# amolrpatil21/PorQua

Measured on AMD Instinct MI355X. Metric: QPs solved/sec (rebalance dates) at N=1000 assets, 1-8 GPU; x vs host CPU, higher is better.
Workload: dtype f64; 1 GPU; config3: long-only min-variance (P=2*Pearson cov, budget + box [0,1]), daily rebalance; n_assets=1000, window=252, dates_per_gpu=4749, global_batch=4749, parallelism=dates-sharded x1

## Files before the change

porqua_amd/csrc/common.h:

```cpp
#pragma once
#include <hip/hip_runtime.h>
#include <stdint.h>

#ifndef PQ_DEVFN
#define PQ_DEVFN __device__ __forceinline__
#endif

namespace pq {

typedef double f64x4 __attribute__((ext_vector_type(4)));

constexpr int TB = 64;
constexpr int KC = 16;
constexpr int LDW = 80;
constexpr int STAGE = KC * LDW;
constexpr int NTHR = 256;

struct Acc {
  f64x4 c[2][2];
  __device__ __forceinline__ void zero() {
#pragma unroll
    for (int m = 0; m < 2; ++m)
#pragma unroll
      for (int n = 0; n < 2; ++n) c[m][n] = f64x4{0.0, 0.0, 0.0, 0.0};
// ... 60 lines not shown
  for (int e = 0; e < 4; ++e) S[(k + e) * LDW + i] = s.v[e];
}

enum { MODE_KI = 0, MODE_IK = 1 };

template <int MA, int MB>
__device__ __forceinline__ void stage_load(Stage4& sa, Stage4& sb, const double* GA, int64_t lda,
                                           int a_i0, const double* GB, int64_t ldb, int b_j0,
                                           int k0, int ka0, int kb0) {
  if (MA == MODE_KI) load_ki(sa, GA, lda, ka0 + k0, a_i0); else load_ik(sa, GA, lda, ka0 + k0, a_i0);
  if (MB == MODE_KI) load_ki(sb, GB, ldb, kb0 + k0, b_j0); else load_ik(sb, GB, ldb, kb0 + k0, b_j0);
}
template <int MA, int MB>
__device__ __forceinline__ void stage_store(const Stage4& sa, const Stage4& sb, double* SA, double* SB) {
  if (MA == MODE_KI) store_ki(sa, SA); else store_ik(sa, SA);
  if (MB == MODE_KI) store_ki(sb, SB); else store_ik(sb, SB);
}

template <int MA, int MB>
__device__ void gemm_stream(Acc& acc, double* lds, const double* GA, int64_t lda, int a_i0, int ka0,
                            const double* GB, int64_t ldb, int b_j0, int kb0, int K) {
  if (K <= 0) return;
  Stage4 ra, rb;
  __syncthreads();
  stage_load<MA, MB>(ra, rb, GA, lda, a_i0, GB, ldb, b_j0, 0, ka0, kb0);
  stage_store<MA, MB>(ra, rb, lds, lds + STAGE);
  __syncthreads();
  int buf = 0;
  for (int k0 = 0; k0 < K; k0 += KC) {
    const bool more = (k0 + KC) < K;
    if (more) stage_load<MA, MB>(ra, rb, GA, lda, a_i0, GB, ldb, b_j0, k0 + KC, ka0, kb0);
    mma_lds(acc, lds + buf * 2 * STAGE, lds + buf * 2 * STAGE + STAGE, KC);
    if (more) stage_store<MA, MB>(ra, rb, lds + (buf ^ 1) * 2 * STAGE, lds + (buf ^ 1) * 2 * STAGE + STAGE);
    __syncthreads();
    buf ^= 1;
  }
}

__device__ __forceinline__ void acc_to_lds(const Acc& acc, double* T, int ldt, double alpha) {
#pragma unroll
  for (int m = 0; m < 2; ++m)
#pragma unroll
    for (int n = 0; n < 2; ++n)
#pragma unroll
      for (int r = 0; r < 4; ++r) T[acc_row(m, r) * ldt + acc_col(n)] = alpha * acc.c[m][n][r];
}
__device__ __forceinline__ void acc_to_lds_T(const Acc& acc, double* S, double alpha) {
#pragma unroll
  for (int m = 0; m < 2; ++m)
#pragma unroll
    for (int n = 0; n < 2; ++n)
#pragma unroll
      for (int r = 0; r < 4; ++r) S[acc_col(n) * LDW + acc_row(m, r)] = alpha * acc.c[m][n][r];
}

__device__ __forceinline__ void acc_store(const Acc& acc, double* G, int64_t ld, int row0, int col0) {
#pragma unroll
  for (int m = 0; m < 2; ++m)
#pragma unroll
    for (int n = 0; n < 2; ++n)
#pragma unroll
      for (int r = 0; r < 4; ++r)
        G[(int64_t)(row0 + acc_row(m, r)) * ld + col0 + acc_col(n)] = acc.c[m][n][r];
}
__device__ __forceinline__ void acc_store_T(const Acc& acc, double* G, int64_t ld, int row0, int col0) {
#pragma unroll
  for (int m = 0; m < 2; ++m)
#pragma unroll
    for (int n = 0; n < 2; ++n)
#pragma unroll
      for (int r = 0; r < 4; ++r)
        G[(int64_t)(row0 + acc_col(n)) * ld + col0 + acc_row(m, r)] = acc.c[m][n][r];
}

__device__ __forceinline__ int loop_zero() {
  int z;
  asm volatile("s_mov_b32 %0, 0" : "=s"(z));
  return z;
}

__device__ __forceinline__ double readlane_f64(double v, int lane) {
  const int lo = __builtin_amdgcn_readlane(__double2loint(v), lane);
  const int hi = __builtin_amdgcn_readlane(__double2hiint(v), lane);
  return __hiloint2double(hi, lo);
}

template <int K>
__device__ __forceinline__ double row_bcast16_k(double v) {
  const int lo = __builtin_amdgcn_update_dpp(0, __double2loint(v), 0x150 + K, 0xF, 0xF, false);
  const int hi = __builtin_amdgcn_update_dpp(0, __double2hiint(v), 0x150 + K, 0xF, 0xF, false);
  return __hiloint2double(hi, lo);
}
__device__ __forceinline__ double row_bcast16(double v, int k) {
  switch (k) {
    case 0: return row_bcast16_k<0>(v);
    case 1: return row_bcast16_k<1>(v);
    case 2: return row_bcast16_k<2>(v);
    case 3: return row_bcast16_k<3>(v);
    case 4: return row_bcast16_k<4>(v);
    case 5: return row_bcast16_k<5>(v);
    case 6: return row_bcast16_k<6>(v);
    case 7: return row_bcast16_k<7>(v);
    case 8: return row_bcast16_k<8>(v);
    case 9: return row_bcast16_k<9>(v);
    case 10: return row_bcast16_k<10>(v);
    case 11: return row_bcast16_k<11>(v);
    case 12: return row_bcast16_k<12>(v);
    case 13: return row_bcast16_k<13>(v);
    case 14: return row_bcast16_k<14>(v);
    default: return row_bcast16_k<15>(v);
  }
}


__device__ __forceinline__ int wave_chol_inv16(double (&A)[4], double (&Bv)[4], const int l) {
  const int cc = l & 15, gg = l >> 4;
  int bad = 0;
#pragma unroll
  for (int kk = 0; kk < 16; ++kk) {
    const int src = ((kk & 3) << 4);
    const double akk = A[kk >> 2];
    const double piv = readlane_f64(akk, src | kk);
    const double rowk = __shfl(akk, src | cc, 64);
    const double bkr = __shfl(Bv[kk >> 2], src | cc, 64);
    double colv[4];
#pragma unroll
    for (int q = 0; q < 4; ++q) colv[q] = row_bcast16(A[q], kk);
    if (!(piv > 0.0) || !isfinite(piv)) bad = 1;
    double rs = __builtin_amdgcn_rsq(piv);
    rs = rs * fma(-0.5 * piv * rs, rs, 1.5);
    rs = rs * fma(-0.5 * piv * rs, rs, 1.5);
    const double bk = bkr * rs;
    const double lck = cc > kk ? rowk * rs : 0.0;
#pragma unroll
    for (int q = 0; q < 4; ++q) {
      if (4 * q + 3 < kk) continue;
      const int r = gg + 4 * q;
      const double lrk = colv[q] * rs;
      const double lrt = r > kk ? lrk : 0.0;
      const double upd = fma(-lrt, lck, A[q]);
      A[q] = (cc == kk && r >= kk) ? lrk : upd;
      const double bu = fma(-lrt, bk, Bv[q]);
      Bv[q] = r == kk ? bk : bu;
    }
  }
  return bad;
}
__device__ __forceinline__ int wave_chol_inv16(double (&A)[4], double (&Bv)[4]) {
  return wave_chol_inv16(A, Bv, lane_id());
}

__device__ __forceinline__ int xcd_slot(int g, int N) {
  const int x = g & 7, q = N >> 3, r = N & 7;
  return (x < r ? x * (q + 1) : r * (q + 1) + (x - r) * q) + (g >> 3);
}

template <int W>
__device__ __forceinline__ double lanes_sum(double v) {
  static_assert(W >= 2 && W <= 64 && (W & (W - 1)) == 0, "a power of two, at most the wave");
#pragma unroll
  for (int o = W / 2; o > 0; o >>= 1) v += __shfl_xor(v, o, 64);
  return v;
}
template <int W>
__device__ __forceinline__ double lanes_max(double v) {
  static_assert(W >= 2 && W <= 64 && (W & (W - 1)) == 0, "a power of two, at most the wave");
#pragma unroll
  for (int o = W / 2; o > 0; o >>= 1) v = fmax(v, __shfl_xor(v, o, 64));
  return v;
}
__device__ __forceinline__ double wave_sum(double v) { return lanes_sum<64>(v); }
__device__ __forceinline__ double wave_max(double v) { return lanes_max<64>(v); }

__device__ __forceinline__ double block_sum(double v, double* red) {
  v = wave_sum(v);
  const int nw = blockDim.x >> 6;
  __syncthreads();
  if (lane_id() == 0) red[wave_id()] = v;
  __syncthreads();
  double s = 0.0;
  for (int w = 0; w < nw; ++w) s += red[w];
  return s;
}
__device__ __forceinline__ double block_max(double v, double* red) {
  v = wave_max(v);
  const int nw = blockDim.x >> 6;
  __syncthreads();
  if (lane_id() == 0) red[wave_id()] = v;
  __syncthreads();
  double s = red[0];
  for (int w = 1; w < nw; ++w) s = fmax(s, red[w]);
  return s;
}

}
```

porqua_amd/csrc/pg_record.h:

```cpp
#pragma once
#include "common.h"
#include "../../include/porqua_hip.h"

namespace pq {

constexpr int PGR = PQ_PG_RECORD;
enum : int {
  R_K = 0, R_MA = 1, R_NZB = 2, R_STATE = 3, R_ROUNDS = 4, R_SC = 5,
  R_FORMED = 6, R_REUSE = 7,
  R_ACT = 64, R_LAM = 128, R_DA = 192, R_SOL = 256, R_AL = 288,
  R_W = 320, R_NFX = 321, R_FIX = 324, R_FIXV = 332, R_FXL = 340,
  R_GFORM = 348,
  R_KB = 349,
  R_LIST = 352, R_CNT = 360
};
constexpr int PG_NBUCKET = 6;
constexpr int PG_BIGB = 5;
__device__ __forceinline__ unsigned long long pg_count(const double* rec, int bk) {
  return reinterpret_cast<const unsigned long long*>(rec + R_CNT)[bk];
}
__device__ __forceinline__ int pg_listed(const double* rec, int bk, int i) {
  return (int)rec[(int64_t)i * PGR + R_LIST + bk];
}
int resident_grid(const void* kernel, int block, int B);
__device__ __forceinline__ int pg_bucket(int kb) {
  return kb <= 48 ? 0 : kb <= 64 ? 1 : kb <= 80 ? 2 : kb <= 96 ? 3 : 4;
}
constexpr int PG_KMAX = 128;
constexpr int PG_KBIG = 256;
constexpr int PG_MGMAX = 32;
constexpr int PG_WMB = 8;
constexpr int PG_WG_MAX = 24;
static_assert(R_FXL + PG_WMB <= R_GFORM && R_KB < R_LIST && R_LIST + 6 <= R_CNT && R_CNT + 6 <= PQ_PG_RECORD,
              "PQ_PG_RECORD too small");

struct PGWork {
  double *xs, *xb, *g, *Px, *rF, *solx, *pxb, *U;
  int *Fl, *fl, *posF;
  __device__ __forceinline__ PGWork(const pq_state& st, int b, int ld) {
    double* W = st.work + (int64_t)b * st.work_stride;
    xs = W;
    xb = W + ld;
    g = W + 2 * (int64_t)ld;
    Px = W + 3 * (int64_t)ld;
    Fl = reinterpret_cast<int*>(W + 4 * (int64_t)ld);
    posF = Fl + ld;
    rF = W + 5 * (int64_t)ld;
    solx = W + 6 * (int64_t)ld;
    pxb = W + 7 * (int64_t)ld;
    U = W + 8 * (int64_t)ld;
    fl = reinterpret_cast<int*>(U + (int64_t)st.mg_pad * ld);
  }
};

__device__ __forceinline__ int pk(int r, int c) { return ((r * (r + 1)) >> 1) + c; }

}

int pq_pg_solve_rt_launch(int nbmax, int B, hipStream_t str, const pq_problem* pb, pq_state* st, double* rec,
                          const pq_settings* s, int ldk);
int pq_pg_wide_launch(const pq_lowrank* lr, const pq_problem* pb, pq_state* st, double* rec, const pq_settings* s,
                      const pq_pg_wide* wd, hipStream_t stream);
```

porqua_amd/csrc/polish_g.hip:

```cpp
#include <cstdlib>
#include <mutex>

#include "polish_dev.h"
#include "capi_util.h"
#include "pg_record.h"

namespace pq {


__global__ __launch_bounds__(PT) void k_pg_init(pq_lowrank lr, pq_problem pb, pq_state st, double* rec,
                                                pq_settings s) {
  __shared__ double red[16];
  const int b = blockIdx.x;
  const int t = threadIdx.x;
  double* R = rec + (int64_t)b * PGR;
  const int st0 = st.status[b];
  if (st0 != PQ_SOLVED && st0 != PQ_MAX_ITER) {
    if (t == 0) R[R_STATE] = PQ_PG_SKIP;
    return;
  }
  const int n = pb.n, ld = pb.ld, mg = pb.mg;
  const double ps = pb.p_scale ? pb.p_scale[b] : 1.0;
  const double pd = pb.p_diag ? pb.p_diag[b] : 0.0;
  const double psw = ps * (lr.w_scale ? lr.w_scale[b] : 1.0);
// ... 2047 lines not shown
    o[PQ_OUT_OBJ] = 0.5 * xpx + qx;
    o[PQ_OUT_PRIM] = fmax(pres, 0.0);
    o[PQ_OUT_DUAL] = dres;
    o[PQ_OUT_GAP] = fabs(xpx + qx + gapb);
    o[PQ_OUT_RHO] = st.rho[b];
    o[PQ_OUT_NFREE] = R[R_K];
    o[PQ_OUT_ROUNDS] = R[R_ROUNDS];
    st.status[b] = PQ_SOLVED;
    R[R_STATE] = PQ_PG_DONE;
  }
}

}

extern "C" int pq_polish_grouped_init(const pq_lowrank* lr, const pq_problem* pb, pq_state* st, double* rec,
                                      const pq_settings* s, void* stream) {
  PQ_CHECK_ARG(lr && pb && st && s && rec, "pq_polish_grouped_init: null argument");
  PQ_CHECK_ARG(lr->dg && lr->panel && lr->rows && lr->tlen, "pq_polish_grouped_init: window (with dg) missing");
  PQ_CHECK_ARG(pb->mg >= 0 && pb->mg <= pq::PG_MGMAX && (pb->mg == 0 || (pb->Cg && pb->lg && pb->ug)),
               "pq_polish_grouped_init: needs 0 <= mg <= %d general rows", pq::PG_MGMAX);
  PQ_CHECK_ARG(st->work && st->work_stride >= PQ_WORK_DOUBLES(pb->ld, st->mg_pad),
               "pq_polish_grouped_init: work buffer too small");
  if (pb->batch <= 0) return 0;
  hipLaunchKernelGGL(pq::k_pg_init, dim3(pb->batch), dim3(pq::PT), 0, (hipStream_t)stream, *lr, *pb, *st, rec, *s);
  PQ_CHECK_LAUNCH("pq_polish_grouped_init");
  return 0;
}

namespace pq {
struct PgSide {
  static constexpr int NS = 7;
  bool ok = false;
  hipStream_t s[NS];
  hipEvent_t fork, join[NS];
};
static PgSide* pg_side() {
  static PgSide sides[64];
  static std::mutex mu;
  int dev = 0;
  if (hipGetDevice(&dev) != hipSuccess || dev < 0 || dev >= 64) return nullptr;
  std::lock_guard<std::mutex> lock(mu);
  PgSide& p = sides[dev];
  if (!p.ok) {
    bool good = hipEventCreateWithFlags(&p.fork, hipEventDisableTiming) == hipSuccess;
    for (int i = 0; i < PgSide::NS && good; ++i)
      good = hipStreamCreateWithFlags(&p.s[i], hipStreamNonBlocking) == hipSuccess &&
             hipEventCreateWithFlags(&p.join[i], hipEventDisableTiming) == hipSuccess;
    if (!good) {
      (void)hipGetLastError();
      return nullptr;
    }
    p.ok = true;
  }
  return &p;
}

static int group_form_min() {
  static const int v = [] {
    const char* e = getenv("PQ_PG_GFORM");
    return e ? atoi(e) : 2;
  }();
  return v;
}

static int group_form_big_min() {
  static const int v = [] {
    const char* e = getenv("PQ_PG_GFORM_BIG");
    return e ? atoi(e) : 2;
  }();
  return v;
}

static int pg_big() {
  static const int v = [] {
    const char* e = getenv("PQ_PG_BIG");
    return e ? atoi(e) : 1;
  }();
  return v;
}

static int solve_rt() {
  static const int v = [] {
    const char* e = getenv("PQ_PG_RT");
    return e ? atoi(e) : 4;
  }();
  return v;
}

static int solve_waves(int bucket) {
  static const int forced = [] {
    const char* e = getenv("PQ_PG_SOLVE_NW");
    const int v = e ? atoi(e) : 0;
    return v == 1 || v == 2 || v == 4 ? v : 0;
  }();
  static const int def[5] = {2, 2, 4, 4, 4};
  return forced ? forced : def[bucket];
}

template <int KS>
static void launch_solve_ks(int nw, int B, hipStream_t str, const pq_problem* pb, pq_state* st, double* rec,
                            const pq_settings* s, int ldk, int klo) {
  const int inner = s->polish_inner > 0 ? s->polish_inner : 0;
  if (nw == 1)
    hipLaunchKernelGGL((k_pg_solve<KS, 1>), dim3(resident_grid((const void*)k_pg_solve<KS, 1>, 64, B)), dim3(64), 0,
                       str, *pb, *st, rec, *s, ldk, klo, inner);
  else if (nw == 2)
    hipLaunchKernelGGL((k_pg_solve<KS, 2>), dim3(resident_grid((const void*)k_pg_solve<KS, 2>, 128, B)), dim3(128),
                       0, str, *pb, *st, rec, *s, ldk, klo, inner);
  else
    hipLaunchKernelGGL((k_pg_solve<KS, 4>), dim3(resident_grid((const void*)k_pg_solve<KS, 4>, 256, B)), dim3(256),
                       0, str, *pb, *st, rec, *s, ldk, klo, inner);
}
static void launch_solve(int bucket, int nw, int B, hipStream_t str, const pq_problem* pb, pq_state* st,
                         double* rec, const pq_settings* s, int ldk, int klo) {
  switch (bucket) {
    case 0: launch_solve_ks<48>(nw, B, str, pb, st, rec, s, ldk, klo); break;
    case 1: launch_solve_ks<64>(nw, B, str, pb, st, rec, s, ldk, klo); break;
    case 2: launch_solve_ks<80>(nw, B, str, pb, st, rec, s, ldk, klo); break;
    case 3: launch_solve_ks<96>(nw, B, str, pb, st, rec, s, ldk, klo); break;
    default: launch_solve_ks<128>(nw, B, str, pb, st, rec, s, ldk, klo); break;
  }
}
}

extern "C" int pq_polish_grouped_round(const pq_lowrank* lr, const pq_problem* pb, pq_state* st, double* rec,
                                       int32_t ldk, const int32_t* gdates, int32_t ngroups, const int32_t* urows,
                                       const int32_t* ucnt, const int32_t* uoff, int32_t umax, const pq_settings* s,
                                       double* pass_scratch, const pq_pg_wide* wide, void* stream) {
  PQ_CHECK_ARG(lr && pb && st && s && rec && pass_scratch, "pq_polish_grouped_round: null argument");
  static_assert(pq::QSCR == pq::GB_OFF && pq::GB_END == PQ_PG_PASS_SCRATCH, "PQ_PG_PASS_SCRATCH out of date");
  PQ_CHECK_ARG(gdates && urows && ucnt && uoff && umax > 0 && umax <= pq::QU,
               "pq_polish_grouped_round: group plan missing (umax <= %d)", pq::QU);
  PQ_CHECK_ARG(pb->n % 2 == 0 && lr->ldp % 2 == 0, "pq_polish_grouped_round: needs even n and panel stride");
  PQ_CHECK_ARG(pb->mg >= 0 && pb->mg <= pq::PG_MGMAX, "pq_polish_grouped_round: mg <= %d", pq::PG_MGMAX);
  PQ_CHECK_ARG(st->K && ldk >= 64 && st->K_stride >= (int64_t)ldk * ldk,
               "pq_polish_grouped_round: K scratch (ldk x ldk per problem) too small");
  if (pb->batch <= 0 || ngroups <= 0) return 0;
  hipStream_t str = (hipStream_t)stream;
  const int B = pb->batch;
  const int kmax = ldk < pq::PG_KMAX ? ldk : pq::PG_KMAX;
  const int kbig = (pq::pg_big() && ldk > kmax) ? (ldk < pq::PG_KBIG ? ldk : pq::PG_KBIG) : kmax;
  hipLaunchKernelGGL(pq::k_pg_setup, dim3(B), dim3(pq::PT), 0, str, *pb, *st, rec, kmax, wide ? 1 : 0, kbig);
  const dim3 gsplit(ngroups * pq::QS);
  hipLaunchKernelGGL(pq::k_pg_passA<0>, gsplit, dim3(pq::QT), 0, str, *lr, *pb, *st, rec, gdates, urows, ucnt, uoff,
                     umax, pass_scratch);
  hipLaunchKernelGGL(pq::k_pg_passB<0>, gsplit, dim3(pq::QT), 0, str, *lr, *pb, *st, rec, gdates, urows, ucnt, uoff,
                     umax, pass_scratch);
  hipLaunchKernelGGL(pq::k_pg_post<0>, dim3(B), dim3(pq::PPT), 0, str, *lr, *pb, *st, rec, *s, gdates, ngroups,
                     pass_scratch);
  if (pq::group_form_min() > 0)
    hipLaunchKernelGGL(pq::k_pg_form_grp, dim3(ngroups), dim3(pq::FT), 0, str, *lr, *pb, *st, rec, gdates, urows,
                       ucnt, umax, pass_scratch, pq::group_form_min());
  hipLaunchKernelGGL(pq::k_pg_form<pq::PG_KMAX>, dim3(B), dim3(pq::FT), 0, str, *lr, *pb, *st, rec, ldk, gdates, ngroups, urows,
                     ucnt, uoff, umax, pass_scratch);
  pq::PgSide* side = pq::pg_side();
  int used = 0;
  if (side && hipEventRecord(side->fork, str) != hipSuccess) side = nullptr;
  auto on = [&](int i) -> hipStream_t {
    if (!side || hipStreamWaitEvent(side->s[i], side->fork, 0) != hipSuccess) return str;
    used |= 1 << i;
    return side->s[i];
  };
  if (kbig > kmax) {
    static_assert(pq::PG_KBIG == 256, "k_pg_form<PG_KBIG> tiling");
    const hipStream_t sb = on(6);
    if (pq::group_form_big_min() > 0 && lr->mu == nullptr)
      hipLaunchKernelGGL(pq::k_pg_form_grp_big, dim3(ngroups * pq::GBS), dim3(pq::FT), 0, sb, *lr, *pb, *st, rec,
                         gdates, urows, ucnt, umax, pass_scratch, pq::group_form_big_min());
    hipLaunchKernelGGL(pq::k_pg_form<pq::PG_KBIG>, dim3(pq::resident_grid((const void*)pq::k_pg_form<pq::PG_KBIG>,
                                                                          pq::FT, B)),
                       dim3(pq::FT), 0, sb, *lr, *pb, *st, rec, ldk, gdates, ngroups, urows, ucnt, uoff, umax,
                       pass_scratch);
    hipLaunchKernelGGL(pq::k_pg_big, dim3(pq::resident_grid((const void*)pq::k_pg_big, pq::PT, B)), dim3(pq::PT), 0,
                       sb, *lr, *pb, *st, rec, *s, ldk, kmax);
  }
  const int nrt = pq::solve_rt() <= 0 ? 0 : (pq::solve_rt() >= 4 ? 4 : 3);
  for (int i = 4; i >= nrt; --i) {
    static const int KSB[5] = {48, 64, 80, 96, 128};
    if (i >= 2 && kmax <= KSB[i - 1]) continue;
    pq::launch_solve(i, pq::solve_waves(i), B, on(i), pb, st, rec, s, ldk, i ? KSB[i - 1] : 0);
  }
  if (nrt > 0 && pq_pg_solve_rt_launch(nrt + 2, B, on(1), pb, st, rec, s, ldk)) return -1;
  if (wide && pq_pg_wide_launch(lr, pb, st, rec, s, wide, on(5))) return -1;
  for (int i = 0; side && i < pq::PgSide::NS; ++i)
    if ((used & (1 << i)) && (hipEventRecord(side->join[i], side->s[i]) != hipSuccess ||
                              hipStreamWaitEvent(str, side->join[i], 0) != hipSuccess)) {
      pq::set_error("pq_polish_grouped_round: joining the solve streams failed");
      return -2;
    }
  hipLaunchKernelGGL(pq::k_pg_passA<1>, gsplit, dim3(pq::QT), 0, str, *lr, *pb, *st, rec, gdates, urows, ucnt, uoff,
                     umax, pass_scratch);
  hipLaunchKernelGGL(pq::k_pg_passB<1>, gsplit, dim3(pq::QT), 0, str, *lr, *pb, *st, rec, gdates, urows, ucnt, uoff,
                     umax, pass_scratch);
  hipLaunchKernelGGL(pq::k_pg_post<1>, dim3(B), dim3(pq::PPT), 0, str, *lr, *pb, *st, rec, *s, gdates, ngroups,
                     pass_scratch);
  PQ_CHECK_LAUNCH("pq_polish_grouped_round");
  return 0;
}

int pq::resident_grid(const void* kernel, int block, int B) {
  struct Entry { const void* k; int dev, n; };
  static Entry cache[64];
  static int used = 0;
  static std::mutex mu;
  int dev = 0;
  if (hipGetDevice(&dev) != hipSuccess) return B;
  std::lock_guard<std::mutex> lock(mu);
  for (int i = 0; i < used; ++i)
    if (cache[i].k == kernel && cache[i].dev == dev) return cache[i].n < B ? cache[i].n : B;
  int per = 0, cus = 0;
  if (hipOccupancyMaxActiveBlocksPerMultiprocessor(&per, kernel, block, 0) != hipSuccess ||
      hipDeviceGetAttribute(&cus, hipDeviceAttributeMultiprocessorCount, dev) != hipSuccess || per <= 0 || cus <= 0) {
    (void)hipGetLastError();
    return B;
  }
  const int n = per * cus;
  if (used < 64) cache[used++] = Entry{kernel, dev, n};
  return n < B ? n : B;
}
```

porqua_amd/csrc/polish_rt.hip:

```cpp
#include <cstdlib>

#include "polish_dev.h"
#include "pg_record.h"

namespace pq {
namespace {

constexpr int RT_WMA = 8;

__device__ constexpr int ti(int I, int J) { return I * (I + 1) / 2 + J; }

__device__ __forceinline__ double sum_g(double v) {
  v += __shfl_xor(v, 16, 64);
  v += __shfl_xor(v, 32, 64);
  return v;
}

template <int NB>
PQ_DEVFN void rt_load(f64x4 (&S)[NB * (NB + 1) / 2], const double* K, int ldk, const int* s_map, int k,
                      double delta, const double* xF, double* px) {
  const int l = (threadIdx.x + loop_zero()) & 63, c16 = l & 15, g = l >> 4;
  const int nbk = (k + 15) >> 4;
#pragma unroll
  for (int I = 0; I < NB; ++I) {
    if (I < nbk) {
      const int r = 16 * I + c16;
      const int mr = s_map[r < k ? r : 0];
#pragma unroll
      for (int J = 0; J <= I; ++J)
#pragma unroll
        for (int q = 0; q < 4; ++q) {
          const int c = 16 * J + g + 4 * q;
          S[ti(I, J)][q] = K[s_map[c < k ? c : 0] * ldk + mr];
        }
    }
  }
  double pr[NB];
#pragma unroll
  for (int I = 0; I < NB; ++I) pr[I] = 0.0;
#pragma unroll
  for (int J = 0; J < NB; ++J) {
    double pc[4] = {0.0, 0.0, 0.0, 0.0};
    if (J < nbk) {
#pragma unroll
      for (int I = J; I < NB; ++I) {
        if (I < nbk) {
          const int r = 16 * I + c16;
          const bool rv = r < k;
          const double xr = rv ? xF[r] : 0.0;
#pragma unroll
          for (int q = 0; q < 4; ++q) {
            const int c = 16 * J + g + 4 * q;
            const bool cv = c < k;
            const double v = (rv && cv) ? S[ti(I, J)][q] : 0.0;
            pr[I] = fma(v, cv ? xF[c] : 0.0, pr[I]);
            if (I > J) pc[q] = fma(v, xr, pc[q]);
            S[ti(I, J)][q] = (r == c) ? (rv ? v + delta : 1.0) : v;
          }
        } else {
#pragma unroll
          for (int q = 0; q < 4; ++q) S[ti(I, J)][q] = 0.0;
        }
      }
    } else {
#pragma unroll
      for (int I = J; I < NB; ++I)
#pragma unroll
        for (int q = 0; q < 4; ++q) S[ti(I, J)][q] = (I == J && c16 == g + 4 * q) ? 1.0 : 0.0;
    }
#pragma unroll
    for (int q = 0; q < 4; ++q) pc[q] = lanes_sum<16>(pc[q]);
    if (c16 == 0) {
#pragma unroll
      for (int q = 0; q < 4; ++q) px[16 * J + g + 4 * q] = pc[q];
    }
  }
  __syncthreads();
#pragma unroll
  for (int I = 0; I < NB; ++I) {
    const double v = sum_g(pr[I]);
    if (g == 0) px[16 * I + c16] += v;
  }
  __syncthreads();
}

template <int NB>
PQ_DEVFN int rt_potrf(f64x4 (&S)[NB * (NB + 1) / 2], int k, double* tsc) {
  const int nbk = (k + 15) >> 4;
#pragma unroll
  for (int J = 0; J < NB; ++J) {
    if (J < nbk) {
      const int l = (threadIdx.x + loop_zero()) & 63, c16 = l & 15, g = l >> 4;
      double A[4], Bv[4];
#pragma unroll
      for (int q = 0; q < 4; ++q) {
        A[q] = S[ti(J, J)][q];
        Bv[q] = (g + 4 * q == c16) ? 1.0 : 0.0;
      }
      if (wave_chol_inv16(A, Bv, l)) return J + 1;
#pragma unroll
      for (int q = 0; q < 4; ++q) tsc[(g + 4 * q) * 17 + c16] = Bv[q];
      __syncthreads();
#pragma unroll
      for (int q = 0; q < 4; ++q) S[ti(J, J)][q] = tsc[c16 * 17 + g + 4 * q];
      __syncthreads();
#pragma unroll
      for (int I = J + 1; I < NB; ++I) {
        if (I < nbk) {
          f64x4 acc = f64x4{0.0, 0.0, 0.0, 0.0};
#pragma unroll
          for (int s4 = 0; s4 < 4; ++s4)
            acc = __builtin_amdgcn_mfma_f64_16x16x4f64(S[ti(J, J)][s4], S[ti(I, J)][s4], acc, 0, 0, 0);
          S[ti(I, J)] = acc;
        }
      }
#pragma unroll
      for (int Jp = J + 1; Jp < NB; ++Jp) {
#pragma unroll
        for (int I = Jp; I < NB; ++I) {
          if (I < nbk) {
            f64x4 acc = S[ti(I, Jp)];
#pragma unroll
            for (int s4 = 0; s4 < 4; ++s4)
              acc = __builtin_amdgcn_mfma_f64_16x16x4f64(-S[ti(Jp, J)][s4], S[ti(I, J)][s4], acc, 0, 0, 0);
            S[ti(I, Jp)] = acc;
          }
        }
      }
    }
  }
  return 0;
}

template <int NB>
PQ_DEVFN void rt_fwd(const f64x4 (&S)[NB * (NB + 1) / 2], int k, const double* b, double* y) {
  const int l = (threadIdx.x + loop_zero()) & 63, c16 = l & 15, g = l >> 4;
  const int nbk = (k + 15) >> 4;
#pragma unroll
  for (int J = 0; J < NB; ++J) {
    if (J < nbk) {
      double part = 0.0;
#pragma unroll
      for (int K = 0; K < J; ++K)
#pragma unroll
        for (int q = 0; q < 4; ++q) part = fma(S[ti(J, K)][q], y[16 * K + g + 4 * q], part);
      part = sum_g(part);
      const double rj = b[16 * J + c16] - part;
      double p2 = 0.0;
#pragma unroll
      for (int q = 0; q < 4; ++q) p2 = fma(S[ti(J, J)][q], __shfl(rj, g + 4 * q, 64), p2);
      p2 = sum_g(p2);
      if (g == 0) y[16 * J + c16] = p2;
      __syncthreads();
    }
  }
}

template <int NB>
PQ_DEVFN void rt_bwd(const f64x4 (&S)[NB * (NB + 1) / 2], int k, const double* y, double* x, double* tv) {
  const int l = (threadIdx.x + loop_zero()) & 63, c16 = l & 15, g = l >> 4;
  const int nbk = (k + 15) >> 4;
#pragma unroll
  for (int J = NB - 1; J >= 0; --J) {
    if (J < nbk) {
      double a[4] = {0.0, 0.0, 0.0, 0.0};
#pragma unroll
      for (int I = J + 1; I < NB; ++I) {
        if (I < nbk) {
          const double xi = x[16 * I + c16];
#pragma unroll
          for (int q = 0; q < 4; ++q) a[q] = fma(S[ti(I, J)][q], xi, a[q]);
        }
      }
      if (J + 1 < nbk) {
#pragma unroll
        for (int q = 0; q < 4; ++q) a[q] = lanes_sum<16>(a[q]);
      }
      if (c16 == 0) {
#pragma unroll
        for (int q = 0; q < 4; ++q) tv[g + 4 * q] = y[16 * J + g + 4 * q] - a[q];
      }
      __syncthreads();
      const double rr = tv[c16];
#pragma unroll
      for (int q = 0; q < 4; ++q) a[q] = lanes_sum<16>(S[ti(J, J)][q] * rr);
      if (c16 == 0) {
#pragma unroll
        for (int q = 0; q < 4; ++q) x[16 * J + g + 4 * q] = a[q];
      }
      __syncthreads();
    }
  }
}

}

constexpr int RT_KS = 96;
struct RtLds {
  double *xF, *rx, *t1, *t2, *px, *vv, *tsc, *Sm, *lamv, *wl, *rl, *dAv;
  int *s_map, *s_m2, *s_f2, *s_vp, *s_vi, *s_al, *s_flag;
};

template <int NB>
__device__ __forceinline__ void rt_solve_date(int b, const pq_problem& pb, const pq_state& st, double* rec,
                                              const pq_settings& s, int ldk, int klo, int inner, const RtLds& L_) {
  constexpr int KS = 16 * NB;
  constexpr int NT = NB * (NB + 1) / 2;
  static_assert(KS <= RT_KS, "rt_solve_date: bucket beyond the LDS sizing");
  double *xF = L_.xF, *rx = L_.rx, *t1 = L_.t1, *t2 = L_.t2, *px = L_.px, *vv = L_.vv, *tsc = L_.tsc;
  double *Sm = L_.Sm, *lamv = L_.lamv, *wl = L_.wl, *rl = L_.rl, *dAv = L_.dAv;
  int *s_map = L_.s_map, *s_m2 = L_.s_m2, *s_f2 = L_.s_f2, *s_vp = L_.s_vp, *s_vi = L_.s_vi, *s_al = L_.s_al;
  int& s_flag = *L_.s_flag;
  double* R = rec + (int64_t)b * PGR;
  if (R[R_STATE] != PQ_PG_PENDING || R[R_W] != 0.0) return;
  const int kb = (int)R[R_KB];
  if (kb <= klo || kb > KS) return;
  int k = kb;
  const int ma = (int)R[R_MA];
  const int t = threadIdx.x;
  if (ma > RT_WMA) {
    if (t == 0) R[R_STATE] = PQ_PG_FALLBACK;
    return;
  }
  const int n = pb.n, ld = pb.ld;
  const double* Cg = pb.Cg ? pb.Cg + (int64_t)b * pb.Cg_stride : nullptr;
  PGWork wk(st, b, ld);
  const double sc = R[R_SC];
  const double delta = s.delta * sc;
  const double* K = st.K + (int64_t)b * st.K_stride;
  const bool reuse = R[R_REUSE] != 0.0;
  for (int p = t; p < KS; p += 64) {
    s_map[p] = p < k ? (reuse ? wk.posF[wk.Fl[p]] : p) : 0;
    xF[p] = p < k ? wk.solx[p] : 0.0;
  }
  if (t < ma) {
    s_al[t] = (int)R[R_AL + t];
    lamv[t] = R[R_SOL + t];
    dAv[t] = R[R_DA + t];
  }
  const bool has_box = pb.lb != nullptr;
  const double* lb = has_box ? pb.lb + (int64_t)b * pb.box_stride : nullptr;
  const double* ub = has_box ? pb.ub + (int64_t)b * pb.box_stride : nullptr;
  __syncthreads();
#ifdef PQ_PROFILE
  long long t_last_ = wall_clock64();
#define RSTAMP(k_)                                                         \
  do {                                                                     \
    __syncthreads();                                                       \
    if (t == 0) { const long long n_ = wall_clock64(); R[8 + (k_)] += (double)(n_ - t_last_); t_last_ = n_; } \
  } while (0)
#else
#define RSTAMP(k_) do { } while (0)
#endif
  f64x4 S[NT];
  for (int it_in = 0;; ++it_in) {
    const int l = threadIdx.x + loop_zero();
    rt_load<NB>(S, K, ldk, s_map, k, delta, xF, px);
    RSTAMP(0);
    if (rt_potrf<NB>(S, k, tsc)) {
      if (l == 0) R[R_STATE] = PQ_PG_FALLBACK;
      return;
    }
    RSTAMP(1);
    for (int a = 0; a < ma; ++a) {
      const double* cr = Cg + (int64_t)s_al[a] * ld;
      for (int p = l; p < KS; p += 64) t1[p] = p < k ? cr[wk.Fl[p]] : 0.0;
      __syncthreads();
      rt_fwd<NB>(S, k, t1, t2);
      for (int p = l; p < k; p += 64) wk.U[(int64_t)a * ld + p] = t2[p];
      __syncthreads();
    }
    for (int e = 0; e < ma * ma; ++e) {
      const int ii = e / ma, jj = e % ma;
      if (jj > ii) continue;
      const double* ui = wk.U + (int64_t)ii * ld;
      const double* uj = wk.U + (int64_t)jj * ld;
      double sum = 0.0;
      for (int p = l; p < k; p += 64) sum += ui[p] * uj[p];
      sum = wave_sum(sum);
      if (l == 0) Sm[ii * RT_WMA + jj] = sum + (ii == jj ? delta : 0.0);
    }
    __syncthreads();
    if (l == 0) {
      int sbad = 0;
      for (int c = 0; c < ma && !sbad; ++c) {
        double d = Sm[c * RT_WMA + c];
        for (int m = 0; m < c; ++m) d -= Sm[c * RT_WMA + m] * Sm[c * RT_WMA + m];
        if (!(d > 0.0) || !isfinite(d)) { sbad = 1; break; }
        d = sqrt(d);
        Sm[c * RT_WMA + c] = d;
        for (int r = c + 1; r < ma; ++r) {
          double v = Sm[r * RT_WMA + c];
          for (int m = 0; m < c; ++m) v -= Sm[r * RT_WMA + m] * Sm[c * RT_WMA + m];
          Sm[r * RT_WMA + c] = v / d;
        }
      }
      s_flag = sbad;
    }
    __syncthreads();
    if (s_flag) {
      if (l == 0) R[R_STATE] = PQ_PG_FALLBACK;
      return;
    }
    RSTAMP(2);
    for (int itr = 0; itr < s.refine_iters; ++itr) {
      if (itr > 0) {
        for (int p = l; p < k; p += 64) {
          double sum = 0.0;
#pragma unroll 8
          for (int qq = 0; qq < k; ++qq) sum = fma(K[(int64_t)s_map[qq] * ldk + s_map[p]], xF[qq], sum);
          px[p] = sum;
        }
      }
      for (int a = 0; a < ma; ++a) {
        const double* cr = Cg + (int64_t)s_al[a] * ld;
        double sum = 0.0;
        for (int p = l; p < k; p += 64) sum += cr[wk.Fl[p]] * xF[p];
        sum = wave_sum(sum);
        if (l == 0) {
          const double v = dAv[a] - sum;
          rl[a] = fabs(v) <= 1e-14 * (1.0 + fabs(dAv[a]) + fabs(sum)) ? 0.0 : v;
        }
      }
      __syncthreads();
      double rm = 0.0;
      for (int p = l; p < KS; p += 64) {
        double v = 0.0;
        if (p < k) {
          v = wk.rF[p] - px[p];
          const int fp = wk.Fl[p];
          for (int a = 0; a < ma; ++a) v -= Cg[(int64_t)s_al[a] * ld + fp] * lamv[a];
        }
        rx[p] = v;
        rm = fmax(rm, fabs(v));
      }
      if (l < ma) rm = fmax(rm, fabs(rl[l]));
      __syncthreads();
      RSTAMP(3);
      if (wave_max(rm) <= 1e-13 * sc) break;
      rt_fwd<NB>(S, k, rx, t2);
      for (int a = 0; a < ma; ++a) {
        const double* ua = wk.U + (int64_t)a * ld;
        double sum = 0.0;
        for (int p = l; p < k; p += 64) sum += ua[p] * t2[p];
        sum = wave_sum(sum);
        if (l == 0) wl[a] = sum - rl[a];
      }
      __syncthreads();
      if (l == 0) {
        for (int ii = 0; ii < ma; ++ii) {
          double v = wl[ii];
          for (int jj = 0; jj < ii; ++jj) v -= Sm[ii * RT_WMA + jj] * wl[jj];
          wl[ii] = v / Sm[ii * RT_WMA + ii];
        }
        for (int ii = ma - 1; ii >= 0; --ii) {
          double v = wl[ii];
          for (int jj = ii + 1; jj < ma; ++jj) v -= Sm[jj * RT_WMA + ii] * wl[jj];
          wl[ii] = v / Sm[ii * RT_WMA + ii];
        }
      }
      __syncthreads();
      for (int p = l; p < KS; p += 64) {
        double v = p < k ? t2[p] : 0.0;
        for (int a = 0; a < ma; ++a) v -= (p < k ? wk.U[(int64_t)a * ld + p] : 0.0) * wl[a];
        t1[p] = v;
      }
      __syncthreads();
      rt_bwd<NB>(S, k, t1, t2, rx);
      for (int p = l; p < k; p += 64) xF[p] += t2[p];
      if (l < ma) lamv[l] += wl[l];
      __syncthreads();
      RSTAMP(4);
    }
    if (it_in >= inner || !has_box) break;
    {
      int nk = 0, nv = 0;
      for (int p0 = 0; p0 < k; p0 += 64) {
        const int p = p0 + l;
        int f = 0, i = 0;
        double v = 0.0;
        if (p < k) {
          i = wk.Fl[p];
          const double xi = xF[p];
          if (!isinf(lb[i]) && xi < lb[i] - 1e-12 * (1.0 + fabs(lb[i]))) { f = 1; v = lb[i]; }
          else if (!isinf(ub[i]) && xi > ub[i] + 1e-12 * (1.0 + fabs(ub[i]))) { f = 2; v = ub[i]; }
        }
        const unsigned long long mv = __ballot(p < k && f != 0);
        const unsigned long long mk = __ballot(p < k && f == 0);
        const unsigned long long below = (1ull << l) - 1ull;
        if (p < k && f != 0) {
          const int j = nv + __popcll(mv & below);
          s_vp[j] = s_map[p];
          s_vi[j] = 4 * i + f;
          vv[j] = v;
        } else if (p < k) {
          const int j = nk + __popcll(mk & below);
          s_m2[j] = s_map[p];
          s_f2[j] = i;
          t1[j] = xF[p];
          t2[j] = wk.rF[p];
        }
        nv += __popcll(mv);
        nk += __popcll(mk);
      }
      __syncthreads();
#ifdef PQ_PROFILE
      if (t == 0) {
        R[20] += 1.0;
        R[21] += (nv > 0 && nv < k) ? 1.0 : 0.0;
        R[22] += (nv < k) ? (double)nv : 0.0;
        R[24] += (double)k;
      }
#endif
      if (nv == 0 || nv == k) break;
      const int k2 = k - nv;
      for (int p = l; p < KS; p += 64) {
        if (p < k2) {
          const int mp = s_m2[p];
          double r = t2[p];
          for (int j = 0; j < nv; ++j)
            if (vv[j] != 0.0) r = fma(-K[(int64_t)mp * ldk + s_vp[j]], vv[j], r);
          wk.rF[p] = r;
          wk.Fl[p] = s_f2[p];
          s_map[p] = mp;
          xF[p] = t1[p];
        } else {
          s_map[p] = 0;
          xF[p] = 0.0;
        }
      }
      for (int j = l; j < nv; j += 64) {
        const int i = s_vi[j] >> 2;
        wk.fl[i] = s_vi[j] & 3;
        wk.xb[i] = vv[j];
      }
      for (int a = 0; a < ma; ++a) {
        const double* cr = Cg + (int64_t)s_al[a] * ld;
        double sum = 0.0;
        for (int j = l; j < nv; j += 64) sum += cr[s_vi[j] >> 2] * vv[j];
        sum = wave_sum(sum);
        if (l == 0) dAv[a] -= sum;
      }
      if (l == 0) R[R_K] = k2;
      k = k2;
      __syncthreads();
    }
  }
  for (int ii = t; ii < n; ii += 64) wk.xs[ii] = wk.xb[ii];
  __syncthreads();
  for (int p = t; p < k; p += 64) {
    wk.xs[wk.Fl[p]] = xF[p];
    wk.solx[p] = xF[p];
  }
  R[R_LAM + t] = 0.0;
  __syncthreads();
  if (t < ma) {
    R[R_LAM + s_al[t]] = lamv[t];
    R[R_SOL + t] = lamv[t];
  }
  RSTAMP(5);
#undef RSTAMP
}

__global__ __launch_bounds__(64) __attribute__((amdgpu_waves_per_eu(2, 2)))
void k_pg_solve_rt(pq_problem pb, pq_state st, double* rec, pq_settings s, int ldk, int inner, int nbmax) {
  __shared__ double xF[RT_KS], rx[RT_KS], t1[RT_KS], t2[RT_KS], px[RT_KS], vv[RT_KS];
  __shared__ double tsc[16 * 17];
  __shared__ double Sm[RT_WMA * RT_WMA], lamv[RT_WMA], wl[RT_WMA], rl[RT_WMA], dAv[RT_WMA];
  __shared__ int s_map[RT_KS], s_m2[RT_KS], s_f2[RT_KS], s_vp[RT_KS], s_vi[RT_KS];
  __shared__ int s_al[RT_WMA];
  __shared__ int s_flag;
  const RtLds L_{xF, rx, t1, t2, px, vv, tsc, Sm, lamv, wl, rl, dAv, s_map, s_m2, s_f2, s_vp, s_vi, s_al, &s_flag};
  const int B = pb.batch;
  const int sel = blockIdx.x / B, i = blockIdx.x - sel * B;
  const int nb = nbmax - sel;
  const int bk = pg_bucket(16 * nb);
  if ((unsigned long long)i >= reinterpret_cast<const unsigned long long*>(rec + R_CNT)[bk]) return;
  const int b = (int)rec[(int64_t)i * PGR + R_LIST + bk];
  switch (nb) {
    case 6: rt_solve_date<6>(b, pb, st, rec, s, ldk, 80, inner, L_); break;
    case 5: rt_solve_date<5>(b, pb, st, rec, s, ldk, 64, inner, L_); break;
    case 4: rt_solve_date<4>(b, pb, st, rec, s, ldk, 48, inner, L_); break;
    default: rt_solve_date<3>(b, pb, st, rec, s, ldk, 0, inner, L_); break;
  }
}

}

int pq_pg_solve_rt_launch(int nbmax, int B, hipStream_t str, const pq_problem* pb, pq_state* st, double* rec,
                          const pq_settings* s, int ldk) {
  if (nbmax < 3 || nbmax > 6) return -1;
  const int inner = s->polish_inner > 0 ? s->polish_inner : 0;
  hipLaunchKernelGGL(pq::k_pg_solve_rt, dim3((nbmax - 2) * B), dim3(64), 0, str, *pb, *st, rec, *s, ldk, inner,
                     nbmax);
  return 0;
}
```

Before: 746,100 QPs/s.

## Extend register-tiled polish solver to 7-8 block buckets with pipelined loads

```diff
diff --git a/porqua_amd/csrc/common.h b/porqua_amd/csrc/common.h
--- a/porqua_amd/csrc/common.h
+++ b/porqua_amd/csrc/common.h
@@ -166,6 +166,12 @@
 __device__ __forceinline__ double readlane_f64(double v, int lane) {
   const int lo = __builtin_amdgcn_readlane(__double2loint(v), lane);
   const int hi = __builtin_amdgcn_readlane(__double2hiint(v), lane);
+  return __hiloint2double(hi, lo);
+}
+
+__device__ __forceinline__ double lane_read(double v, int lane) {
+  const int lo = __builtin_amdgcn_ds_bpermute(lane << 2, __double2loint(v));
+  const int hi = __builtin_amdgcn_ds_bpermute(lane << 2, __double2hiint(v));
   return __hiloint2double(hi, lo);
 }
 
@@ -205,8 +211,8 @@
     const int src = ((kk & 3) << 4);
     const double akk = A[kk >> 2];
     const double piv = readlane_f64(akk, src | kk);
-    const double rowk = __shfl(akk, src | cc, 64);
-    const double bkr = __shfl(Bv[kk >> 2], src | cc, 64);
+    const double rowk = lane_read(akk, src | cc);
+    const double bkr = lane_read(Bv[kk >> 2], src | cc);
     double colv[4];
 #pragma unroll
     for (int q = 0; q < 4; ++q) colv[q] = row_bcast16(A[q], kk);
diff --git a/porqua_amd/csrc/pg_record.h b/porqua_amd/csrc/pg_record.h
--- a/porqua_amd/csrc/pg_record.h
+++ b/porqua_amd/csrc/pg_record.h
@@ -57,7 +57,7 @@
 
 }
 
-int pq_pg_solve_rt_launch(int nbmax, int B, hipStream_t str, const pq_problem* pb, pq_state* st, double* rec,
+int pq_pg_solve_rt_launch(int nbhi, int nblo, int B, hipStream_t str, const pq_problem* pb, pq_state* st, double* rec,
                           const pq_settings* s, int ldk);
 int pq_pg_wide_launch(const pq_lowrank* lr, const pq_problem* pb, pq_state* st, double* rec, const pq_settings* s,
                       const pq_pg_wide* wd, hipStream_t stream);
diff --git a/porqua_amd/csrc/polish_g.hip b/porqua_amd/csrc/polish_g.hip
--- a/porqua_amd/csrc/polish_g.hip
+++ b/porqua_amd/csrc/polish_g.hip
@@ -2153,7 +2153,7 @@
 static int solve_rt() {
   static const int v = [] {
     const char* e = getenv("PQ_PG_RT");
-    return e ? atoi(e) : 4;
+    return e ? atoi(e) : 5;
   }();
   return v;
 }
@@ -2245,13 +2245,15 @@
     hipLaunchKernelGGL(pq::k_pg_big, dim3(pq::resident_grid((const void*)pq::k_pg_big, pq::PT, B)), dim3(pq::PT), 0,
                        sb, *lr, *pb, *st, rec, *s, ldk, kmax);
   }
-  const int nrt = pq::solve_rt() <= 0 ? 0 : (pq::solve_rt() >= 4 ? 4 : 3);
+  const int vrt = pq::solve_rt();
+  const int nrt = vrt <= 0 ? 0 : (vrt >= 5 ? 5 : (vrt == 4 ? 4 : 3));
   for (int i = 4; i >= nrt; --i) {
     static const int KSB[5] = {48, 64, 80, 96, 128};
     if (i >= 2 && kmax <= KSB[i - 1]) continue;
     pq::launch_solve(i, pq::solve_waves(i), B, on(i), pb, st, rec, s, ldk, i ? KSB[i - 1] : 0);
   }
-  if (nrt > 0 && pq_pg_solve_rt_launch(nrt + 2, B, on(1), pb, st, rec, s, ldk)) return -1;
+  if (nrt == 5 && kmax > 96 && pq_pg_solve_rt_launch(8, 7, B, on(4), pb, st, rec, s, ldk)) return -1;
+  if (nrt > 0 && pq_pg_solve_rt_launch(nrt >= 4 ? 6 : 5, 3, B, on(1), pb, st, rec, s, ldk)) return -1;
   if (wide && pq_pg_wide_launch(lr, pb, st, rec, s, wide, on(5))) return -1;
   for (int i = 0; side && i < pq::PgSide::NS; ++i)
     if ((used & (1 << i)) && (hipEventRecord(side->join[i], side->s[i]) != hipSuccess ||
diff --git a/porqua_amd/csrc/polish_rt.hip b/porqua_amd/csrc/polish_rt.hip
--- a/porqua_amd/csrc/polish_rt.hip
+++ b/porqua_amd/csrc/polish_rt.hip
@@ -10,122 +10,130 @@
 
 __device__ constexpr int ti(int I, int J) { return I * (I + 1) / 2 + J; }
 
-__device__ __forceinline__ double sum_g(double v) {
-  v += __shfl_xor(v, 16, 64);
-  v += __shfl_xor(v, 32, 64);
+template <int W>
+__device__ __forceinline__ double rt_sum(double v, int l) {
+#pragma unroll
+  for (int o = W / 2; o > 0; o >>= 1) v += lane_read(v, l ^ o);
   return v;
+}
+__device__ __forceinline__ double rt_max(double v, int l) {
+#pragma unroll
+  for (int o = 32; o > 0; o >>= 1) v = fmax(v, lane_read(v, l ^ o));
+  return v;
+}
+__device__ __forceinline__ double sum_g(double v, int l) {
+  v += lane_read(v, l ^ 16);
+  v += lane_read(v, l ^ 32);
+  return v;
+}
+
+template <int NB, int J>
+PQ_DEVFN void rt_issue(f64x4 (&S)[NB * (NB + 1) / 2], const char* Kb, int ldk, const int* s_map, int k) {
+  const int l = (threadIdx.x + loop_zero()) & 63, c16 = l & 15, g = l >> 4;
+  unsigned oc[4];
+#pragma unroll
+  for (int q = 0; q < 4; ++q) {
+    const int c = 16 * J + g + 4 * q;
+    oc[q] = ((unsigned)s_map[c < k ? c : 0] * (unsigned)ldk) << 3;
+  }
+#pragma unroll
+  for (int I = J; I < NB; ++I) {
+    const int r = 16 * I + c16;
+    const unsigned orow = (unsigned)s_map[r < k ? r : 0] << 3;
+#pragma unroll
+    for (int q = 0; q < 4; ++q) S[ti(I, J)][q] = *reinterpret_cast<const double*>(Kb + (oc[q] + orow));
+  }
+}
+
+template <int NB, int J>
+PQ_DEVFN void rt_load_col(f64x4 (&S)[NB * (NB + 1) / 2], const char* Kb, int ldk, const int* s_map, int k,
+                          double delta, const double* xF, double* px, double (&pr)[NB]) {
+  if constexpr (J < NB) {
+    if constexpr (J + 1 < NB) rt_issue<NB, J + 1>(S, Kb, ldk, s_map, k);
+    __builtin_amdgcn_sched_barrier(0);
+    const int l = (threadIdx.x + loop_zero()) & 63, c16 = l & 15, g = l >> 4;
+    double pc[4] = {0.0, 0.0, 0.0, 0.0}, xc[4];
+#pragma unroll
+    for (int q = 0; q < 4; ++q) xc[q] = xF[16 * J + g + 4 * q];
+#pragma unroll
+    for (int I = J; I < NB; ++I) {
+      const int r = 16 * I + c16;
+      const bool rv = r < k;
+      const double xr = xF[r];
+#pragma unroll
+      for (int q = 0; q < 4; ++q) {
+        const int c = 16 * J + g + 4 * q;
+        const bool cv = c < k;
+        const double v = (rv && cv) ? S[ti(I, J)][q] : 0.0;
+        pr[I] = fma(v, xc[q], pr[I]);
+        if (I > J) pc[q] = fma(v, xr, pc[q]);
+        S[ti(I, J)][q] = (r == c) ? (rv ? v + delta : 1.0) : v;
+      }
+    }
+#pragma unroll
+    for (int q = 0; q < 4; ++q) pc[q] = rt_sum<16>(pc[q], l);
+    if (c16 == 0) {
+#pragma unroll
+      for (int q = 0; q < 4; ++q) px[16 * J + g + 4 * q] = pc[q];
+    }
+    rt_load_col<NB, J + 1>(S, Kb, ldk, s_map, k, delta, xF, px, pr);
+  }
 }
 
 template <int NB>
 PQ_DEVFN void rt_load(f64x4 (&S)[NB * (NB + 1) / 2], const double* K, int ldk, const int* s_map, int k,
                       double delta, const double* xF, double* px) {
+  const char* Kb = reinterpret_cast<const char*>(K);
+  double pr[NB];
+#pragma unroll
+  for (int I = 0; I < NB; ++I) pr[I] = 0.0;
+  rt_issue<NB, 0>(S, Kb, ldk, s_map, k);
+  rt_load_col<NB, 0>(S, Kb, ldk, s_map, k, delta, xF, px, pr);
+  __syncthreads();
   const int l = (threadIdx.x + loop_zero()) & 63, c16 = l & 15, g = l >> 4;
-  const int nbk = (k + 15) >> 4;
 #pragma unroll
   for (int I = 0; I < NB; ++I) {
-    if (I < nbk) {
-      const int r = 16 * I + c16;
-      const int mr = s_map[r < k ? r : 0];
-#pragma unroll
-      for (int J = 0; J <= I; ++J)
-#pragma unroll
-        for (int q = 0; q < 4; ++q) {
-          const int c = 16 * J + g + 4 * q;
-          S[ti(I, J)][q] = K[s_map[c < k ? c : 0] * ldk + mr];
-        }
-    }
-  }
-  double pr[NB];
-#pragma unroll
-  for (int I = 0; I < NB; ++I) pr[I] = 0.0;
+    const double v = sum_g(pr[I], l);
+    if (g == 0) px[16 * I + c16] += v;
+  }
+  __syncthreads();
+}
+
+template <int NB>
+PQ_DEVFN int rt_potrf(f64x4 (&S)[NB * (NB + 1) / 2], double* tsc) {
 #pragma unroll
   for (int J = 0; J < NB; ++J) {
-    double pc[4] = {0.0, 0.0, 0.0, 0.0};
-    if (J < nbk) {
-#pragma unroll
-      for (int I = J; I < NB; ++I) {
-        if (I < nbk) {
-          const int r = 16 * I + c16;
-          const bool rv = r < k;
-          const double xr = rv ? xF[r] : 0.0;
-#pragma unroll
-          for (int q = 0; q < 4; ++q) {
-            const int c = 16 * J + g + 4 * q;
-            const bool cv = c < k;
-            const double v = (rv && cv) ? S[ti(I, J)][q] : 0.0;
-            pr[I] = fma(v, cv ? xF[c] : 0.0, pr[I]);
-            if (I > J) pc[q] = fma(v, xr, pc[q]);
-            S[ti(I, J)][q] = (r == c) ? (rv ? v + delta : 1.0) : v;
-          }
-        } else {
-#pragma unroll
-          for (int q = 0; q < 4; ++q) S[ti(I, J)][q] = 0.0;
-        }
-      }
-    } else {
-#pragma unroll
-      for (int I = J; I < NB; ++I)
-#pragma unroll
-        for (int q = 0; q < 4; ++q) S[ti(I, J)][q] = (I == J && c16 == g + 4 * q) ? 1.0 : 0.0;
-    }
-#pragma unroll
-    for (int q = 0; q < 4; ++q) pc[q] = lanes_sum<16>(pc[q]);
-    if (c16 == 0) {
-#pragma unroll
-      for (int q = 0; q < 4; ++q) px[16 * J + g + 4 * q] = pc[q];
-    }
-  }
-  __syncthreads();
-#pragma unroll
-  for (int I = 0; I < NB; ++I) {
-    const double v = sum_g(pr[I]);
-    if (g == 0) px[16 * I + c16] += v;
-  }
-  __syncthreads();
-}
-
-template <int NB>
-PQ_DEVFN int rt_potrf(f64x4 (&S)[NB * (NB + 1) / 2], int k, double* tsc) {
-  const int nbk = (k + 15) >> 4;
-#pragma unroll
-  for (int J = 0; J < NB; ++J) {
-    if (J < nbk) {
-      const int l = (threadIdx.x + loop_zero()) & 63, c16 = l & 15, g = l >> 4;
-      double A[4], Bv[4];
-#pragma unroll
-      for (int q = 0; q < 4; ++q) {
-        A[q] = S[ti(J, J)][q];
-        Bv[q] = (g + 4 * q == c16) ? 1.0 : 0.0;
-      }
-      if (wave_chol_inv16(A, Bv, l)) return J + 1;
-#pragma unroll
-      for (int q = 0; q < 4; ++q) tsc[(g + 4 * q) * 17 + c16] = Bv[q];
-      __syncthreads();
-#pragma unroll
-      for (int q = 0; q < 4; ++q) S[ti(J, J)][q] = tsc[c16 * 17 + g + 4 * q];
-      __syncthreads();
-#pragma unroll
-      for (int I = J + 1; I < NB; ++I) {
-        if (I < nbk) {
-          f64x4 acc = f64x4{0.0, 0.0, 0.0, 0.0};
-#pragma unroll
-          for (int s4 = 0; s4 < 4; ++s4)
-            acc = __builtin_amdgcn_mfma_f64_16x16x4f64(S[ti(J, J)][s4], S[ti(I, J)][s4], acc, 0, 0, 0);
-          S[ti(I, J)] = acc;
-        }
-      }
-#pragma unroll
-      for (int Jp = J + 1; Jp < NB; ++Jp) {
-#pragma unroll
-        for (int I = Jp; I < NB; ++I) {
-          if (I < nbk) {
-            f64x4 acc = S[ti(I, Jp)];
-#pragma unroll
-            for (int s4 = 0; s4 < 4; ++s4)
-              acc = __builtin_amdgcn_mfma_f64_16x16x4f64(-S[ti(Jp, J)][s4], S[ti(I, J)][s4], acc, 0, 0, 0);
-            S[ti(I, Jp)] = acc;
-          }
-        }
+    const int l = (threadIdx.x + loop_zero()) & 63, c16 = l & 15, g = l >> 4;
+    double A[4], Bv[4];
+#pragma unroll
+    for (int q = 0; q < 4; ++q) {
+      A[q] = S[ti(J, J)][q];
+      Bv[q] = (g + 4 * q == c16) ? 1.0 : 0.0;
+    }
+    if (wave_chol_inv16(A, Bv, l)) return J + 1;
+#pragma unroll
+    for (int q = 0; q < 4; ++q) tsc[(g + 4 * q) * 17 + c16] = Bv[q];
+    __syncthreads();
+#pragma unroll
+    for (int q = 0; q < 4; ++q) S[ti(J, J)][q] = tsc[c16 * 17 + g + 4 * q];
+    __syncthreads();
+#pragma unroll
+    for (int I = J + 1; I < NB; ++I) {
+      f64x4 acc = f64x4{0.0, 0.0, 0.0, 0.0};
+#pragma unroll
+      for (int s4 = 0; s4 < 4; ++s4)
+        acc = __builtin_amdgcn_mfma_f64_16x16x4f64(S[ti(J, J)][s4], S[ti(I, J)][s4], acc, 0, 0, 0);
+      S[ti(I, J)] = acc;
+    }
+#pragma unroll
+    for (int Jp = J + 1; Jp < NB; ++Jp) {
+#pragma unroll
+      for (int I = Jp; I < NB; ++I) {
+        f64x4 acc = S[ti(I, Jp)];
+#pragma unroll
+        for (int s4 = 0; s4 < 4; ++s4)
+          acc = __builtin_amdgcn_mfma_f64_16x16x4f64(S[ti(Jp, J)][s4], S[ti(I, J)][s4], acc, 0, 0, 1);
+        S[ti(I, Jp)] = acc;
       }
     }
   }
@@ -144,12 +152,12 @@
       for (int K = 0; K < J; ++K)
 #pragma unroll
         for (int q = 0; q < 4; ++q) part = fma(S[ti(J, K)][q], y[16 * K + g + 4 * q], part);
-      part = sum_g(part);
+      part = sum_g(part, l);
       const double rj = b[16 * J + c16] - part;
       double p2 = 0.0;
 #pragma unroll
-      for (int q = 0; q < 4; ++q) p2 = fma(S[ti(J, J)][q], __shfl(rj, g + 4 * q, 64), p2);
-      p2 = sum_g(p2);
+      for (int q = 0; q < 4; ++q) p2 = fma(S[ti(J, J)][q], lane_read(rj, g + 4 * q), p2);
+      p2 = sum_g(p2, l);
       if (g == 0) y[16 * J + c16] = p2;
       __syncthreads();
     }
@@ -174,7 +182,7 @@
       }
       if (J + 1 < nbk) {
 #pragma unroll
-        for (int q = 0; q < 4; ++q) a[q] = lanes_sum<16>(a[q]);
+        for (int q = 0; q < 4; ++q) a[q] = rt_sum<16>(a[q], l);
       }
       if (c16 == 0) {
 #pragma unroll
@@ -183,7 +191,7 @@
       __syncthreads();
       const double rr = tv[c16];
 #pragma unroll
-      for (int q = 0; q < 4; ++q) a[q] = lanes_sum<16>(S[ti(J, J)][q] * rr);
+      for (int q = 0; q < 4; ++q) a[q] = rt_sum<16>(S[ti(J, J)][q] * rr, l);
       if (c16 == 0) {
 #pragma unroll
         for (int q = 0; q < 4; ++q) x[16 * J + g + 4 * q] = a[q];
@@ -195,7 +203,7 @@
 
 }
 
-constexpr int RT_KS = 96;
+constexpr int RT_KS = 128;
 struct RtLds {
   double *xF, *rx, *t1, *t2, *px, *vv, *tsc, *Sm, *lamv, *wl, *rl, *dAv;
   int *s_map, *s_m2, *s_f2, *s_vp, *s_vi, *s_al, *s_flag;
@@ -257,7 +265,7 @@
     const int l = threadIdx.x + loop_zero();
     rt_load<NB>(S, K, ldk, s_map, k, delta, xF, px);
     RSTAMP(0);
-    if (rt_potrf<NB>(S, k, tsc)) {
+    if (rt_potrf<NB>(S, tsc)) {
       if (l == 0) R[R_STATE] = PQ_PG_FALLBACK;
       return;
     }
@@ -270,14 +278,13 @@
       for (int p = l; p < k; p += 64) wk.U[(int64_t)a * ld + p] = t2[p];
       __syncthreads();
     }
-    for (int e = 0; e < ma * ma; ++e) {
-      const int ii = e / ma, jj = e % ma;
-      if (jj > ii) continue;
+    for (int ii = 0; ii < ma; ++ii)
+    for (int jj = 0; jj <= ii; ++jj) {
       const double* ui = wk.U + (int64_t)ii * ld;
       const double* uj = wk.U + (int64_t)jj * ld;
       double sum = 0.0;
       for (int p = l; p < k; p += 64) sum += ui[p] * uj[p];
-      sum = wave_sum(sum);
+      sum = rt_sum<64>(sum, l);
       if (l == 0) Sm[ii * RT_WMA + jj] = sum + (ii == jj ? delta : 0.0);
     }
     __syncthreads();
@@ -316,7 +323,7 @@
         const double* cr = Cg + (int64_t)s_al[a] * ld;
         double sum = 0.0;
         for (int p = l; p < k; p += 64) sum += cr[wk.Fl[p]] * xF[p];
-        sum = wave_sum(sum);
+        sum = rt_sum<64>(sum, l);
         if (l == 0) {
           const double v = dAv[a] - sum;
           rl[a] = fabs(v) <= 1e-14 * (1.0 + fabs(dAv[a]) + fabs(sum)) ? 0.0 : v;
@@ -337,13 +344,13 @@
       if (l < ma) rm = fmax(rm, fabs(rl[l]));
       __syncthreads();
       RSTAMP(3);
-      if (wave_max(rm) <= 1e-13 * sc) break;
+      if (rt_max(rm, l) <= 1e-13 * sc) break;
       rt_fwd<NB>(S, k, rx, t2);
       for (int a = 0; a < ma; ++a) {
         const double* ua = wk.U + (int64_t)a * ld;
         double sum = 0.0;
         for (int p = l; p < k; p += 64) sum += ua[p] * t2[p];
-        sum = wave_sum(sum);
+        sum = rt_sum<64>(sum, l);
         if (l == 0) wl[a] = sum - rl[a];
       }
       __syncthreads();
@@ -438,7 +445,7 @@
         const double* cr = Cg + (int64_t)s_al[a] * ld;
         double sum = 0.0;
         for (int j = l; j < nv; j += 64) sum += cr[s_vi[j] >> 2] * vv[j];
-        sum = wave_sum(sum);
+        sum = rt_sum<64>(sum, l);
         if (l == 0) dAv[a] -= sum;
       }
       if (l == 0) R[R_K] = k2;
@@ -446,52 +453,63 @@
       __syncthreads();
     }
   }
-  for (int ii = t; ii < n; ii += 64) wk.xs[ii] = wk.xb[ii];
+  const int te = threadIdx.x + loop_zero();
+  for (int ii = te; ii < n; ii += 64) wk.xs[ii] = wk.xb[ii];
   __syncthreads();
-  for (int p = t; p < k; p += 64) {
+  for (int p = te; p < k; p += 64) {
     wk.xs[wk.Fl[p]] = xF[p];
     wk.solx[p] = xF[p];
   }
-  R[R_LAM + t] = 0.0;
+  R[R_LAM + te] = 0.0;
   __syncthreads();
-  if (t < ma) {
-    R[R_LAM + s_al[t]] = lamv[t];
-    R[R_SOL + t] = lamv[t];
+  if (te < ma) {
+    R[R_LAM + s_al[te]] = lamv[te];
+    R[R_SOL + te] = lamv[te];
   }
   RSTAMP(5);
 #undef RSTAMP
 }
 
-__global__ __launch_bounds__(64) __attribute__((amdgpu_waves_per_eu(2, 2)))
-void k_pg_solve_rt(pq_problem pb, pq_state st, double* rec, pq_settings s, int ldk, int inner, int nbmax) {
-  __shared__ double xF[RT_KS], rx[RT_KS], t1[RT_KS], t2[RT_KS], px[RT_KS], vv[RT_KS];
+template <int NB, int NBLO>
+__device__ __forceinline__ void rt_dispatch(int nb, int b, const pq_problem& pb, const pq_state& st, double* rec,
+                                            const pq_settings& s, int ldk, int inner, const RtLds& L_) {
+  if (nb == NB) rt_solve_date<NB>(b, pb, st, rec, s, ldk, NB > 3 ? 16 * (NB - 1) : 0, inner, L_);
+  else if constexpr (NB > NBLO) rt_dispatch<NB - 1, NBLO>(nb, b, pb, st, rec, s, ldk, inner, L_);
+}
+
+template <int NBHI, int NBLO, int WPE>
+__global__ __launch_bounds__(64) __attribute__((amdgpu_waves_per_eu(WPE, WPE)))
+void k_pg_solve_rt(pq_problem pb, pq_state st, double* rec, pq_settings s, int ldk, int inner) {
+  constexpr int KS = 16 * NBHI;
+  static_assert(NBLO >= 3 && NBLO <= NBHI && KS <= RT_KS, "k_pg_solve_rt: buckets 3..8");
+  __shared__ double xF[KS], rx[KS], t1[KS], t2[KS], px[KS], vv[KS];
   __shared__ double tsc[16 * 17];
   __shared__ double Sm[RT_WMA * RT_WMA], lamv[RT_WMA], wl[RT_WMA], rl[RT_WMA], dAv[RT_WMA];
-  __shared__ int s_map[RT_KS], s_m2[RT_KS], s_f2[RT_KS], s_vp[RT_KS], s_vi[RT_KS];
+  __shared__ int s_map[KS], s_m2[KS], s_f2[KS], s_vp[KS], s_vi[KS];
   __shared__ int s_al[RT_WMA];
   __shared__ int s_flag;
   const RtLds L_{xF, rx, t1, t2, px, vv, tsc, Sm, lamv, wl, rl, dAv, s_map, s_m2, s_f2, s_vp, s_vi, s_al, &s_flag};
   const int B = pb.batch;
   const int sel = blockIdx.x / B, i = blockIdx.x - sel * B;
-  const int nb = nbmax - sel;
+  const int nb = NBHI - sel;
   const int bk = pg_bucket(16 * nb);
-  if ((unsigned long long)i >= reinterpret_cast<const unsigned long long*>(rec + R_CNT)[bk]) return;
-  const int b = (int)rec[(int64_t)i * PGR + R_LIST + bk];
-  switch (nb) {
-    case 6: rt_solve_date<6>(b, pb, st, rec, s, ldk, 80, inner, L_); break;
-    case 5: rt_solve_date<5>(b, pb, st, rec, s, ldk, 64, inner, L_); break;
-    case 4: rt_solve_date<4>(b, pb, st, rec, s, ldk, 48, inner, L_); break;
-    default: rt_solve_date<3>(b, pb, st, rec, s, ldk, 0, inner, L_); break;
-  }
-}
-
-}
-
-int pq_pg_solve_rt_launch(int nbmax, int B, hipStream_t str, const pq_problem* pb, pq_state* st, double* rec,
-                          const pq_settings* s, int ldk) {
-  if (nbmax < 3 || nbmax > 6) return -1;
+  if ((unsigned long long)i >= pg_count(rec, bk)) return;
+  const int b = __builtin_amdgcn_readfirstlane(pg_listed(rec, bk, i));
+  rt_dispatch<NBHI, NBLO>(nb, b, pb, st, rec, s, ldk, inner, L_);
+}
+
+using RtKernel = void (*)(pq_problem, pq_state, double*, pq_settings, int, int);
+
+}
+
+int pq_pg_solve_rt_launch(int nbhi, int nblo, int B, hipStream_t str, const pq_problem* pb, pq_state* st,
+                          double* rec, const pq_settings* s, int ldk) {
+  pq::RtKernel kern = nullptr;
+  if (nbhi == 8 && nblo == 7) kern = pq::k_pg_solve_rt<8, 7, 1>;
+  else if (nbhi == 6 && nblo == 3) kern = pq::k_pg_solve_rt<6, 3, 2>;
+  else if (nbhi == 5 && nblo == 3) kern = pq::k_pg_solve_rt<5, 3, 2>;
+  if (!kern) return -1;
   const int inner = s->polish_inner > 0 ? s->polish_inner : 0;
-  hipLaunchKernelGGL(pq::k_pg_solve_rt, dim3((nbmax - 2) * B), dim3(64), 0, str, *pb, *st, rec, *s, ldk, inner,
-                     nbmax);
+  hipLaunchKernelGGL(kern, dim3((nbhi - nblo + 1) * B), dim3(64), 0, str, *pb, *st, rec, *s, ldk, inner);
   return 0;
 }
```

New measurement: 745,600 QPs/s, median of 2. No clear change (-0.1%).
